# yurimjeon1892/EFGH

Hardware: AMD Instinct MI355X
Metric: frame-pairs/sec EFGHNet fwd+bwd (384x1280 RGB + 64x2048 range), whole job (higher is better)
Workload: dtype f32; 1 GPU; BASELINE.json configs[2]: EFGHNet fwd+bwd with efghloss + gradient all-reduce + fused Adam, synthetic 384x1280 RGB + 131072-point sweep, batch=8 per GPU, random-init weights; global_batch=8, points=131072, parallelism=dp1

## Files before the change

### efgh_amd/_C.py

```python
import ctypes
import os

_HERE = os.path.dirname(os.path.abspath(__file__))
SO_PATH = os.environ.get('EFGH_LIB') or os.path.join(_HERE, 'lib', 'libefgh_hip.so')
_lib = None
ABI_VERSION = 4

c_void_p, c_int, c_int32, c_int64, c_float = (ctypes.c_void_p, ctypes.c_int, ctypes.c_int32,
                                              ctypes.c_int64, ctypes.c_float)


class EfghError(RuntimeError):
    pass


class GemmDesc(ctypes.Structure):
    _fields_ = [
        ('A', c_void_p), ('lda', c_int64), ('C', c_int32), ('T', c_int32), ('mode', c_int32),
        ('B', c_int32), ('Hin', c_int32), ('Win', c_int32), ('Hv', c_int32), ('Wv', c_int32),
        ('sh', c_int32), ('sw', c_int32),
        ('dh', ctypes.c_int8 * 16), ('dw', ctypes.c_int8 * 16),
        ('Ho', c_int32), ('Wo', c_int32), ('osh', c_int32), ('osw', c_int32), ('oh0', c_int32),
        ('ow0', c_int32),
        ('table', c_void_p), ('W', c_void_p), ('N', c_int32), ('M', c_int64), ('M_dev', c_void_p),
        ('bias', c_void_p), ('scale', c_void_p), ('shift', c_void_p),
        ('residual', c_void_p), ('ldr', c_int64),
        ('act', c_int32), ('slope', c_float), ('out', c_void_p), ('ldo', c_int64),
        ('stats', c_void_p),
        ('nbatch', c_int32), ('batch_stride_a', c_int64), ('batch_stride_w', c_int64), ('batch_stride_out', c_int64),
        ('batch_stride_table', c_int32), ('table_alias_mask', c_int32),
        ('stats_mode', c_int32), ('bn_raw', c_void_p), ('bn_ldraw', c_int64), ('bn_y', c_void_p), ('bn_ldy', c_int64),
        ('bn_pscale', c_void_p), ('bn_pshift', c_void_p), ('bn_mean', c_void_p), ('bn_invstd', c_void_p),
        ('bn_act', c_int32), ('bn_slope', c_float),
    ]


class WgradOutDesc(ctypes.Structure):
    _fields_ = [('W', c_void_p), ('N', c_int32), ('T', c_int32), ('C', c_int32), ('Cp', c_int32),
                ('sn', c_int64), ('sc', c_int64), ('st', c_int64), ('taps', c_int32 * 16), ('accumulate', c_int32)]


GUARD_MAX_SEGMENTS = 8
GUARD_RUN = 4096


class GuardState(ctypes.Structure):
    _fields_ = [('sumsq', ctypes.c_double * GUARD_MAX_SEGMENTS), ('sumsq_total', ctypes.c_double), ('norm', ctypes.c_double),
                ('nonfinite', c_int64 * GUARD_MAX_SEGMENTS), ('nonfinite_total', c_int64),
                ('applied', c_int64), ('skipped', c_int64),
                ('coef', c_float), ('scale', c_float), ('bc1', c_float), ('bc2_sqrt', c_float),
                ('skip', c_int32), ('nseg', c_int32)]


class TxnState(ctypes.Structure):
    _fields_ = [('forward_nonfinite', c_int64), ('rolled_back', c_int64), ('vetoed_total', c_int64),
                ('first_bad', c_int32), ('vetoed', c_int32)]


WROTE_OUT = 1


def check_wrote(rc):
    if rc == WROTE_OUT:
        return True
    check(rc)
    return False


def lib():
    global _lib
    if _lib is None:
        if not os.path.exists(SO_PATH):
            raise EfghError(f'{SO_PATH} is missing: run `python -c "import __graft_entry__ as g; '
                            f'g.build()"` (hipcc, gfx950). There is no CPU fallback.')
        import torch
        _lib = ctypes.CDLL(SO_PATH)
        _lib.efgh_last_error.restype = ctypes.c_char_p
        _lib.efgh_version.restype = c_int
        if _lib.efgh_version() != ABI_VERSION:
            got, _lib = _lib.efgh_version(), None
            raise EfghError(f'{SO_PATH} has ABI version {got}, this package binds version {ABI_VERSION} of include/efgh_hip.h: '
                            f'rebuild it (`python -m efgh_amd.build`)')
        _lib.efgh_wino2d_tiles.restype = c_int64
        _lib.efgh_segment_workspace.restype = c_int64
        _lib.efgh_gather_wgrad_workspace.restype = c_int64
        _lib.efgh_plane_wgrad_workspace.restype = c_int64
        _lib.efgh_wino_wgrad_workspace.restype = c_int64
        _lib.efgh_sc_wgrad_workspace.restype = c_int64
        _lib.efgh_c4n4_wgrad_workspace.restype = c_int64
        _lib.efgh_c4_wgrad_workspace.restype = c_int64
        _lib.efgh_thin_wgrad_workspace.restype = c_int64
        _lib.efgh_lattice_hash_capacity.restype = c_int64
        _lib.efgh_lattice_hash_capacity.argtypes = [c_int32]
        _lib.efgh_lattice_workspace_bytes.restype = c_int64
        _lib.efgh_lattice_workspace_bytes.argtypes = [c_int32, c_int32, c_int32]
        _lib.efgh_lattice_part_max_entries.argtypes = [c_int32]
        _lib.efgh_lattice_part_buckets.argtypes = [c_int32]
        _lib.efgh_lattice_part_list_len.restype = c_int64
        _lib.efgh_lattice_part_list_len.argtypes = [c_int32, c_int32]
        _lib.efgh_lattice_part_zeroed_bytes.restype = c_int64
        _lib.efgh_lattice_part_zeroed_bytes.argtypes = [c_int32]
        _lib.efgh_lattice_part_workspace_bytes.restype = c_int64
        _lib.efgh_lattice_part_workspace_bytes.argtypes = [c_int32, c_int32, c_int32, c_int32, c_int32]
        _lib.efgh_lattice_neighbors_r_workspace.restype = c_int64
        _lib.efgh_lattice_neighbors_r_workspace.argtypes = [c_int32, c_int32]
        _lib.efgh_lattice_index_bytes.restype = c_int64
        _lib.efgh_lattice_index_bytes.argtypes = [c_int32, c_int32]
        _lib.efgh_offsets_invert_workspace.restype = c_int64
        _lib.efgh_offsets_invert_workspace.argtypes = [c_int32, c_int32]
        _lib.efgh_slice_bwd_workspace.restype = c_int64
        _lib.efgh_slice_bwd_workspace.argtypes = [c_int32]
        _lib.efgh_grad_guard_workspace.restype = c_int64
        _lib.efgh_grad_guard_workspace.argtypes = [c_int64]
        _lib.efgh_grad_guard_measure.argtypes = [c_void_p, c_int64, ctypes.POINTER(c_int64), c_int32, ctypes.c_double, c_float,
                                                 c_int32, c_float, c_float, c_int32, c_void_p, c_void_p, c_int32, c_void_p]
        _lib.efgh_adam_step_guarded.argtypes = [c_void_p, c_void_p, c_void_p, c_void_p, c_int64, c_float, c_float, c_float,
                                                c_float, c_float, c_void_p, c_void_p]
        _lib.efgh_grad_drain.argtypes = [c_void_p, c_void_p, c_int64, c_int32, c_void_p]
        _lib.efgh_gimg_valid_count.argtypes = [c_void_p, c_void_p, c_int32, c_int64, c_void_p, c_void_p]
        _lib.efgh_txn_snapshot.argtypes = [c_void_p, c_void_p, c_int64, c_void_p, c_void_p, c_int64, c_void_p, c_void_p]
        _lib.efgh_txn_probe.argtypes = [c_void_p, c_void_p, c_int64, c_void_p, c_int32, c_void_p, c_int32, c_int64, c_void_p,
                                        c_void_p]
        _lib.efgh_txn_resolve.argtypes = [c_void_p, c_void_p, c_int64, c_void_p, c_void_p, c_int64, c_void_p, c_void_p, c_float,
                                          c_float, c_void_p]
    return _lib


def check(rc):
    if rc != 0:
        raise EfghError(f'libefgh_hip: rc={rc}: {lib().efgh_last_error().decode()}')


def ptr(t):
    return c_void_p(0 if t is None else t.data_ptr())


_raw_stream = None


def stream_ptr():
    global _raw_stream
    import torch
    if _raw_stream is None:
        get, dev = getattr(torch._C, '_cuda_getCurrentRawStream', None), getattr(torch._C, '_cuda_getDevice', None)
        if get is not None and dev is not None:
            _raw_stream = lambda: get(dev())
        else:
            _raw_stream = lambda: torch.cuda.current_stream().cuda_stream
    return c_void_p(_raw_stream())


def require_cuda(*tensors):
    for t in tensors:
        if t is not None and not t.is_cuda:
            raise EfghError('efgh_amd runs on the GPU through libefgh_hip.so only (got a CPU tensor); '
                            'there is no CPU fallback')


def require_f32(*tensors):
    import torch
    for t in tensors:
        if t is not None and t.dtype != torch.float32:
            raise EfghError('efgh_amd expects float32 tensors, got %s (cast with .float() as iterater.py:29-32 does)' % t.dtype)
```

### efgh_amd/csrc/wgrad.hip

```cpp
#include "common.h"

namespace {

typedef float f32x16 __attribute__((ext_vector_type(16)));
constexpr int TK = 128, TM = 32, LD = 128;

struct WArgs {
    const float *A; int64_t lda;
    int C, T, K;
    unsigned magicC;
    int Hin, Win, Hv, Wv, sh, sw;
    unsigned long long dhpack, dwpack;
    int Ho, Wo, osh, osw, oh0, ow0;
    const int *table;
    const float *G; int64_t ldg;
    int N;
    int tld;
    long long M; int mchunk;
    float *dW;
    long long zstride;
    unsigned kt, nt;
    long long bsA, bsG, bsD;
};

// ... 64 lines not shown
    }
    float4 rg[NGQ], ra[4];
    auto load_step = [&](long long ms) {
        if (TN != 128) {
#pragma unroll
            for (int q = 0; q < NGQ; ++q) {
                long long m = ms + gr0 + GRS * q;
                float4 g = make_float4(0.f, 0.f, 0.f, 0.f);
                if (m < mend && nin) g = *reinterpret_cast<const float4 *>(MODE == 1 ? git[q].g : p.G + m * p.ldg + n0 + gc4);
                rg[q] = g;
                if (MODE == 1) advance(git[q], n0 + gc4);
            }
        }
#pragma unroll
        for (int q = 0; q < 4; ++q) {
            long long m = ms + r0 + 8 * q;
            float4 g = make_float4(0.f, 0.f, 0.f, 0.f), a = g;
            if (m < mend) {
                if (MODE == 1) {
                    if (TN == 128 && nin) g = *reinterpret_cast<const float4 *>(rit[q].g);
                    if (kin && rit[q].rowok && (unsigned)(rit[q].j * p.sw + dw) < (unsigned)p.Win)
                        a = *reinterpret_cast<const float4 *>(rit[q].a);
                } else {
                    long long arow = -1;
                    if (MODE == 0) arow = m;
                    else if (kin) arow = p.table[m * (MODE == 4 ? p.tld : 16) + t];
                    if (TN == 128 && nin) g = *reinterpret_cast<const float4 *>(p.G + m * p.ldg + n0 + c4);
                    if (kin && arow >= 0) a = *reinterpret_cast<const float4 *>(p.A + arow * p.lda + c);
                }
            }
            if (TN == 128) rg[q] = g;
            ra[q] = a;
            if (MODE == 1) advance(rit[q], n0 + c4);
        }
    };

    f32x16 acc[2][TJ];
#pragma unroll
    for (int i = 0; i < 2; ++i)
#pragma unroll
        for (int j = 0; j < TJ; ++j)
#pragma unroll
            for (int r = 0; r < 16; ++r) acc[i][j][r] = 0.f;

    load_step(mbeg);
    for (long long ms = mbeg; ms < mend; ms += TM) {
#pragma unroll
        for (int q = 0; q < 4; ++q)
            *reinterpret_cast<float4 *>(&As[(r0 + 8 * q) * LD + c4]) = ra[q];
#pragma unroll
        for (int q = 0; q < NGQ; ++q)
            *reinterpret_cast<float4 *>(&Gs[(gr0 + GRS * q) * TN + gc4]) = rg[q];
        __syncthreads();
        if (ms + TM < mend) load_step(ms + TM);
#pragma unroll
        for (int mm = 0; mm < TM / 2; ++mm) {
            float g[2], a[TJ];
#pragma unroll
            for (int i = 0; i < 2; ++i) g[i] = Gs[(mm * 2 + lh) * TN + (wn * 2 + i) * 32 + l31];
#pragma unroll
            for (int j = 0; j < TJ; ++j) a[j] = As[(mm * 2 + lh) * LD + (wk * TJ + j) * 32 + l31];
#pragma unroll
            for (int i = 0; i < 2; ++i)
#pragma unroll
                for (int j = 0; j < TJ; ++j)
                    acc[i][j] = __builtin_amdgcn_mfma_f32_32x32x2f32(g[i], a[j], acc[i][j], 0, 0, 0);
        }
        __syncthreads();
    }
#pragma unroll
    for (int i = 0; i < 2; ++i)
#pragma unroll
        for (int j = 0; j < TJ; ++j) {
            const int k = k0 + (wk * TJ + j) * 32 + l31;
            if (k >= p.K) continue;
#pragma unroll
            for (int r = 0; r < 16; ++r) {
                const int n = n0 + (wn * 2 + i) * 32 + (r & 3) + 8 * (r >> 2) + 4 * lh;
                if (n < p.N) p.dW[(long long)n * p.K + k] = acc[i][j][r];
            }
        }
}

typedef efgh_wgrad_out_desc FoldUnpackArgs;

template <bool UNPACK>
__global__ void __launch_bounds__(256) k_fold_splits(const float4 *part, int zs, long long total4, float4 *dst, const FoldUnpackArgs u) {
    __shared__ float4 red[256];
    const int e = threadIdx.x & 15, zl = threadIdx.x >> 4;
    const long long i = (long long)blockIdx.x * 16 + e;
    float4 a = make_float4(0.f, 0.f, 0.f, 0.f), b = a;
    if (i < total4) {
        int z = zl;
        for (; z + 16 < zs; z += 32) {
            const float4 u = part[(long long)z * total4 + i], v = part[(long long)(z + 16) * total4 + i];
            a.x += u.x; a.y += u.y; a.z += u.z; a.w += u.w;
            b.x += v.x; b.y += v.y; b.z += v.z; b.w += v.w;
        }
        if (z < zs) { const float4 u = part[(long long)z * total4 + i]; a.x += u.x; a.y += u.y; a.z += u.z; a.w += u.w; }
        a.x += b.x; a.y += b.y; a.z += b.z; a.w += b.w;
    }
    red[threadIdx.x] = a;
    __syncthreads();
    for (int h = 8; h; h >>= 1) {
        if (zl < h) {
            const float4 o = red[threadIdx.x + h * 16];
            float4 m = red[threadIdx.x];
            m.x += o.x; m.y += o.y; m.z += o.z; m.w += o.w;
            red[threadIdx.x] = m;
        }
        __syncthreads();
    }
    if (zl == 0 && i < total4) {
        if (!UNPACK) { dst[i] = red[e]; return; }
        const float4 v4 = red[e];
        const float v[4] = {v4.x, v4.y, v4.z, v4.w};
        const long long idx = 4 * i;
        const int c0 = (int)(idx % u.Cp); const long long r = idx / u.Cp;
        const int t = (int)(r % u.T), n = (int)(r / u.T);
        if (n >= u.N) return;
        int ti = 0;
#pragma unroll
        for (int q = 0; q < 16; ++q) if (q == t) ti = u.taps[q];
#pragma unroll
        for (int q = 0; q < 4; ++q) {
            if (c0 + q >= u.C) continue;
            float *d = &u.W[n * u.sn + (c0 + q) * u.sc + ti * u.st];
            *d = u.accumulate ? *d + v[q] : v[q];
        }
    }
}

__global__ void k_unpack_weight(const float *__restrict__ Wp, float *__restrict__ W, int N, int T, int C,
                                int Cp, long long sn, long long sc, long long st, const int4 taps0,
                                const int4 taps1, const int4 taps2, const int4 taps3, int accumulate) {
    const int tp[16] = {taps0.x, taps0.y, taps0.z, taps0.w, taps1.x, taps1.y, taps1.z, taps1.w,
                        taps2.x, taps2.y, taps2.z, taps2.w, taps3.x, taps3.y, taps3.z, taps3.w};
    long long total = (long long)N * T * C;
    for (long long i = (long long)blockIdx.x * blockDim.x + threadIdx.x; i < total;
         i += (long long)gridDim.x * blockDim.x) {
        int c = (int)(i % C); long long r = i / C;
        int t = (int)(r % T); int n = (int)(r / T);
        int ti = 0;
#pragma unroll
        for (int q = 0; q < 16; ++q) if (q == t) ti = tp[q];
        float v = Wp[((long long)n * T + t) * Cp + c];
        float *dst = &W[n * sn + c * sc + ti * st];
        *dst = accumulate ? *dst + v : v;
    }
}

__global__ void __launch_bounds__(256)
k_table_scatter_add(const float *__restrict__ src, const int *__restrict__ table, long long M, int T, int C,
                    float *__restrict__ dst) {
    const int c4n = C >> 2;
    long long total = M * T * c4n;
    for (long long i = (long long)blockIdx.x * 256 + threadIdx.x; i < total; i += (long long)gridDim.x * 256) {
        int cq = (int)(i % c4n); long long r = i / c4n;
        int t = (int)(r % T); long long m = r / T;
        int row = table[m * 16 + t];
        if (row < 0) continue;
        float4 v = *reinterpret_cast<const float4 *>(src + (m * T + t) * C + cq * 4);
        float *d = dst + (long long)row * C + cq * 4;
        atomicAdd(d + 0, v.x); atomicAdd(d + 1, v.y); atomicAdd(d + 2, v.z); atomicAdd(d + 3, v.w);
    }
}

}

bool efgh_launch_fold_splits(const float *part, int zs, long long total, float *dst, hipStream_t st, const efgh_wgrad_out_desc *out) {
    const long long total4 = total / 4;
    const unsigned grid = (unsigned)((total4 + 15) / 16);
    if (out && out->W && out->T >= 1 && out->T <= 16 && out->Cp >= out->C && out->Cp % 4 == 0) {
        const long long row = (long long)out->T * out->Cp;
        if (total % row == 0 && total / row >= out->N && total / row < out->N + 4) {
            k_fold_splits<true><<<grid, 256, 0, st>>>((const float4 *)part, zs, total4, (float4 *)dst, *out);
            return true;
        }
    }
    FoldUnpackArgs none = {};
    k_fold_splits<false><<<grid, 256, 0, st>>>((const float4 *)part, zs, total4, (float4 *)dst, none);
    return false;
}

static int gather_wgrad_impl(const efgh_gemm_desc *d, const float *G, int64_t ldg, float *dWp, float *workspace, int nbatch,
                             int64_t bsG, int64_t bsD, const efgh_wgrad_out_desc *out, void *stream_, int tld = 0);


static long long wgrad_chunks(const efgh_gemm_desc *d, int nbatch, long long *chunk_out) {
    const int K = d->T * d->C;
    const int TN = d->N <= 64 ? 64 : 128;
    const long long kt = (K + TK - 1) / TK, nt = (d->N + TN - 1) / TN;
    static const int occ128[3] = {efgh_wg_per_cu((const void *)k_gather_wgrad<0, 128>, 256, 0), efgh_wg_per_cu((const void *)k_gather_wgrad<1, 128>, 256, 0),
                                  efgh_wg_per_cu((const void *)k_gather_wgrad<2, 128>, 256, 0)};
    static const int occ64[3] = {efgh_wg_per_cu((const void *)k_gather_wgrad<0, 64>, 256, 0), efgh_wg_per_cu((const void *)k_gather_wgrad<1, 64>, 256, 0),
                                 efgh_wg_per_cu((const void *)k_gather_wgrad<2, 64>, 256, 0)};
    const int mode = d->mode >= 0 && d->mode <= 2 ? d->mode : 0;
    return efgh_round_chunks(d->M, kt * nt * nbatch, TN == 128 ? occ128[mode] : occ64[mode], TM, 256, (double)nbatch * d->N * K, chunk_out);
}

extern "C" int64_t efgh_gather_wgrad_workspace(const efgh_gemm_desc *d) {
    if (!d || d->C <= 0 || d->T < 1 || d->N < 1 || d->M < 1) return 0;
    const int nbatch = d->nbatch > 1 ? d->nbatch : 1;
    const long long zs = wgrad_chunks(d, nbatch, nullptr);
    return zs > 1 ? zs * nbatch * (int64_t)d->N * d->T * d->C : 0;
}

extern "C" int efgh_gather_wgrad(const efgh_gemm_desc *d, const float *G, int64_t ldg, float *dWp, float *workspace,
                                 const efgh_wgrad_out_desc *out, void *stream_) {
    return gather_wgrad_impl(d, G, ldg, dWp, workspace, 1, 0, 0, out, stream_);
}

extern "C" int efgh_gather_wgrad_batched(const efgh_gemm_desc *d, const float *G, int64_t ldg, int64_t batch_stride_g,
                                         float *dWp, int64_t batch_stride_dw, float *workspace, void *stream_) {
    EFGH_CHECK_ARG(d && d->mode == 0 && d->nbatch >= 1 && d->nbatch <= 65535);
    EFGH_CHECK_ARG(d->batch_stride_a % 4 == 0 && batch_stride_g % 4 == 0 && batch_stride_dw == (int64_t)d->N * d->C);
    return gather_wgrad_impl(d, G, ldg, dWp, workspace, d->nbatch, batch_stride_g, batch_stride_dw, nullptr, stream_);
}

static int gather_wgrad_impl(const efgh_gemm_desc *d, const float *G, int64_t ldg, float *dWp, float *workspace, int nbatch,
                             int64_t bsG, int64_t bsD, const efgh_wgrad_out_desc *out, void *stream_, int tld) {
    hipStream_t st = (hipStream_t)stream_;
    EFGH_CHECK_ARG(d && d->A && G && dWp);
    EFGH_CHECK_ARG(d->C > 0 && d->C % 4 == 0 && d->T >= 1 && (d->T <= 16 || tld > 0) && d->N >= 1 && d->M >= 1);
    EFGH_CHECK_ARG(tld == 0 || (d->mode == 2 && d->table != nullptr && tld >= d->T && nbatch == 1 && !out));
    EFGH_CHECK_ARG(d->lda % 4 == 0 && ldg % 4 == 0 && d->N % 4 == 0);
    EFGH_CHECK_ARG((((uintptr_t)d->A) & 15) == 0 && (((uintptr_t)G) & 15) == 0 && (((uintptr_t)dWp) & 15) == 0);
    EFGH_CHECK_ARG((int64_t)d->T * d->C < 65536 && d->mode >= 0 && d->mode <= 2);
    WArgs a;
    a.A = d->A; a.lda = d->lda; a.C = d->C; a.T = d->T; a.K = d->T * d->C;
    a.magicC = (unsigned)((0x100000000ULL + d->C - 1) / d->C);
    a.Hin = d->Hin; a.Win = d->Win; a.Hv = d->Hv; a.Wv = d->Wv; a.sh = d->sh; a.sw = d->sw;
    a.dhpack = 0; a.dwpack = 0;
    for (int t = 0; t < 16; ++t) {
        int dh = t < d->T ? d->dh[t] : 0, dw = t < d->T ? d->dw[t] : 0;
        a.dhpack |= (unsigned long long)((dh + 8) & 15) << (4 * t);
        a.dwpack |= (unsigned long long)((dw + 8) & 15) << (4 * t);
    }
    a.Ho = d->Ho; a.Wo = d->Wo; a.osh = d->osh; a.osw = d->osw; a.oh0 = d->oh0; a.ow0 = d->ow0;
    a.table = d->table; a.G = G; a.ldg = ldg; a.N = d->N; a.M = d->M;
    a.bsA = nbatch > 1 ? d->batch_stride_a : 0; a.bsG = bsG; a.bsD = bsD; a.tld = tld;
    if (d->mode == 1) EFGH_CHECK_ARG(d->M == (int64_t)d->B * d->Hv * d->Wv && d->osh >= 1 && d->osw >= 1);
    if (d->mode == 2) EFGH_CHECK_ARG(d->table != nullptr);
    const int TN = a.N <= 64 ? 64 : 128;
    const int kt = (a.K + TK - 1) / TK, nt = (a.N + TN - 1) / TN;
    long long chunk = 0;
    const long long zs = wgrad_chunks(d, nbatch, &chunk);
    a.mchunk = (int)chunk;
    EFGH_CHECK_ARG(zs * kt * nt < 0x7fffffffLL);
    a.kt = (unsigned)kt; a.nt = (unsigned)nt;
    const long long plane = (long long)nbatch * a.N * a.K;
    EFGH_CHECK_ARG(zs == 1 || (workspace && (((uintptr_t)workspace) & 15) == 0));
    a.dW = zs > 1 ? workspace : dWp;
    a.zstride = zs > 1 ? plane : 0;
    const dim3 grid((unsigned)(zs * kt * nt), (unsigned)nbatch);
    if (tld > 0) {
        if (TN == 128) k_gather_wgrad<4, 128><<<grid, 256, 0, st>>>(a);
        else k_gather_wgrad<4, 64><<<grid, 256, 0, st>>>(a);
    } else if (TN == 128) {
        if (d->mode == 0) k_gather_wgrad<0, 128><<<grid, 256, 0, st>>>(a);
        else if (d->mode == 1) k_gather_wgrad<1, 128><<<grid, 256, 0, st>>>(a);
        else k_gather_wgrad<2, 128><<<grid, 256, 0, st>>>(a);
    } else {
        if (d->mode == 0) k_gather_wgrad<0, 64><<<grid, 256, 0, st>>>(a);
        else if (d->mode == 1) k_gather_wgrad<1, 64><<<grid, 256, 0, st>>>(a);
        else k_gather_wgrad<2, 64><<<grid, 256, 0, st>>>(a);
    }
    bool wrote = false;
    if (zs > 1) wrote = efgh_launch_fold_splits(workspace, (int)zs, plane, dWp, st, nbatch == 1 ? out : nullptr);
    EFGH_CHECK_LAUNCH();
    return wrote ? EFGH_WROTE_OUT : EFGH_OK;
}

extern "C" int efgh_blur_r_wgrad(const efgh_gemm_desc *d, int32_t ld, const float *G, int64_t ldg, float *dWp, float *workspace,
                                 void *stream_) {
    EFGH_CHECK_ARG(ld > 0);
    const int rc = gather_wgrad_impl(d, G, ldg, dWp, workspace, 1, 0, 0, nullptr, stream_, ld);
    return rc == EFGH_WROTE_OUT ? EFGH_OK : rc;
}

extern "C" int efgh_unpack_weight(const float *Wp, float *W, int32_t N, int32_t T, int32_t C, int32_t Cp,
                                  int64_t sn, int64_t sc, int64_t stt, const int32_t *tapidx, int32_t accumulate,
                                  void *stream_) {
    EFGH_CHECK_ARG(Wp && W && N > 0 && T > 0 && T <= 16 && C > 0 && Cp >= C);
    int tp[16];
    for (int t = 0; t < 16; ++t) tp[t] = (tapidx && t < T) ? tapidx[t] : (t < T ? t : 0);
    long long total = (long long)N * T * C;
    int grid = (int)((total + 255) / 256);
    if (grid > 8192) grid = 8192;
    k_unpack_weight<<<grid, 256, 0, (hipStream_t)stream_>>>(Wp, W, N, T, C, Cp, sn, sc, stt,
                                                           make_int4(tp[0], tp[1], tp[2], tp[3]),
                                                           make_int4(tp[4], tp[5], tp[6], tp[7]),
                                                           make_int4(tp[8], tp[9], tp[10], tp[11]),
                                                           make_int4(tp[12], tp[13], tp[14], tp[15]), accumulate);
    EFGH_CHECK_LAUNCH();
    return EFGH_OK;
}

extern "C" int efgh_table_scatter_add(const float *src, const int32_t *table, int64_t M, int32_t T, int32_t C,
                                      float *dst, void *stream_) {
    EFGH_CHECK_ARG(src && table && dst && M > 0 && T > 0 && T <= 16 && C % 4 == 0);
    long long total = M * T * (C / 4);
    long long g = (total + 255) / 256;
    k_table_scatter_add<<<(int)(g > 16384 ? 16384 : g), 256, 0, (hipStream_t)stream_>>>(src, table, M, T, C, dst);
    EFGH_CHECK_LAUNCH();
    return EFGH_OK;
}

extern "C" int efgh_debug_occupancy(char *out, int32_t cap) {
    EFGH_CHECK_ARG(out && cap > 64);
    snprintf(out, cap, "k_gather_wgrad<0,128> %d  <1,128> %d  <2,128> %d  <0,64> %d  <1,64> %d  <2,64> %d workgroups per CU",
             efgh_wg_per_cu((const void *)k_gather_wgrad<0, 128>, 256, 0), efgh_wg_per_cu((const void *)k_gather_wgrad<1, 128>, 256, 0),
             efgh_wg_per_cu((const void *)k_gather_wgrad<2, 128>, 256, 0), efgh_wg_per_cu((const void *)k_gather_wgrad<0, 64>, 256, 0),
             efgh_wg_per_cu((const void *)k_gather_wgrad<1, 64>, 256, 0), efgh_wg_per_cu((const void *)k_gather_wgrad<2, 64>, 256, 0));
    return EFGH_OK;
}
```

### efgh_amd/ops.py

```python
import ctypes
import os as _os
import threading
import weakref

import torch

from . import _C
from ._C import c_float, c_int32, c_int64, ptr

ACT_NONE, ACT_RELU, ACT_LEAKY = 0, 1, 2


def _L():
    return _C.lib()


def _st():
    return _C.stream_ptr()


def ceil4(n):
    return (n + 3) // 4 * 4


# ... 542 lines not shown
    def regroup():
        return Wp.view(N, S, Ts * C).permute(1, 0, 2).contiguous()
    Wg = _cached(Wp, ('ksplit', S), _ver(Wp), regroup)
    part = _scratch(S * M * N, dev)
    gather_gemm(A, lda, C, Ts, Wg, N, M, part, N, mode=2, table=table, a_off=a_off, batch=(S, 0, N * Ts * C, M * N, Ts),
                flops=flops if flops is not None else 2.0 * M * N * 15 * C, alias_mask=alias_mask)
    b = None
    if bias is not None:
        b = bias if bias.numel() == N else None
        assert b is not None
    _C.check(_L().efgh_fold_planes(ptr(part), c_int32(S), c_int64(M), c_int32(N), ptr(b), c_int32(act), c_float(slope),
                                   _C.c_void_p(out.data_ptr() + 4 * out_off), c_int64(ldo), _st()))


def gather_gemm(A, lda, C, T, Wp, N, M, out, ldo, mode=0, geom=None, table=None, bias=None, scale=None,
                shift=None, residual=None, ldr=0, act=ACT_NONE, slope=0.0, stats=None, a_off=0, out_off=0,
                res_off=0, M_dev=None, flops=None, batch=None, alias_mask=False, bn_bwd=None, pool=False, lazy=None, pre_v=None):
    key = (mode, C, N, T, geom, M, stats is not None, M_dev is not None, batch is not None, pool,
           scale is None and shift is None and residual is None and (bias is None or bias.numel() == N))
    route = gemm_route(*key)
    if (lazy is not None or pre_v is not None) and not (route == 'wino2d' and min(C, N) >= 64):
        raise _C.EfghError('gather_gemm(lazy= / pre_v=) on a launch the 2-D Winograd path does not serve (ask lazy_capable() first)')
    if route == 'blur_r':
        if (geom is not None or batch is not None or M_dev is not None or scale is not None or shift is not None or residual is not None
                or stats is not None or alias_mask or pool or bn_bwd is not None):
            raise _C.EfghError('gather_gemm(mode=MODE_BLUR_R) takes a plain blur launch: bias and activation only')
        blur_r_gemm(A, lda, C, T, Wp, N, M, out, ldo, table, bias=bias, act=act, slope=slope, a_off=a_off, out_off=out_off, flops=flops)
        return None
    if route == 'ksplit':
        return _blur_gemm_ksplit(A, lda, C, Wp, N, M, out, ldo, table, bias, act, slope, a_off, out_off, flops, alias_mask)
    d = _desc(A, lda, C, T, mode, N, M, geom, table, a_off, Wp, out, ldo, out_off, bias, scale, shift, residual, ldr, res_off, act, slope,
              stats, M_dev, batch)
    d.table_alias_mask = 1 if (alias_mask and mode == 2) else 0
    if route == 'sc' and not _sc_aligned(d, lda, ldo, residual, ldr, stats):
        route = gemm_route(*key, aligned=False)
    if pool and route not in ('c4', 'wino2d', 'wino_hpool'):
        raise _C.EfghError('gather_gemm(pool=True) on a launch no pooling epilogue serves (ask pool_fusable() first)')
    ev = _prof_start(PROFILE)
    bn_stats = None
    if route == 'thin':
        if TRACE_THIN is not None:
            TRACE_THIN.append(int(_L().efgh_thin_supported(ctypes.byref(d))))
        _C.check(_L().efgh_thin_gemm(ctypes.byref(d), _st()))
    elif route == 'c4':
        assert lda % 4 == 0
        _C.check((_L().efgh_c4_conv3x3_pooled if pool else _L().efgh_c4_conv3x3)(ctypes.byref(d), _st()))
    elif route == 'sc':
        _C.check(_L().efgh_sc_conv3x3(ctypes.byref(d), _st()))
    elif route == 'wino2d':
        if (bn_bwd is not None and stats is None and BN_BWD_FUSED_2D and out_off == 0 and not pool and bn_bwd.fits(M, N)
                and bn_bwd.y is None and bn_bwd.raw.stride(-2) % 4 == 0):
            rows = _L().efgh_wino2d_stats_rows(c_int32(geom[0]), c_int32(geom[1]), c_int32(geom[2]), c_int32(N))
            bn_stats = _bn_bwd_sums(d, bn_bwd, rows, N, out.device)
        _wino2d_forward(d, A, a_off, lda, C, N, geom, Wp, pool=pool, lazy=lazy, pre_v=pre_v)
    elif route == 'wino_hpool':
        _C.check(_L().efgh_wino_conv3x3_hpool(ctypes.byref(d), ptr(wino_weight(Wp, N, C)), _st()))
    elif route == 'wino':
        if bn_bwd is not None and stats is None and BN_BWD_FUSED and out_off == 0 and bn_bwd.fits(M, N):
            rows = _L().efgh_wino_grid_m(c_int32(geom[0]), c_int32(geom[1]), c_int32(geom[2]))
            bn_stats = _bn_bwd_sums(d, bn_bwd, rows, N, out.device)
        _C.check(_L().efgh_wino_conv3x3(ctypes.byref(d), ptr(wino_weight(Wp, N, C)), _st()))
    else:
        _C.check(_L().efgh_gather_gemm(ctypes.byref(d), _st()))
    if ev is not None:
        _prof_end(ev, route, (mode, M, N, T, C), float(flops) if flops is not None else 2.0 * M * N * T * C, PROFILE, PROFILE_WINO,
                  batched=batch is not None)
    return bn_stats


def _bn_bwd_sums(d, src, rows, N, device):
    part = torch.empty((rows, 2, N), dtype=torch.float32, device=device)
    d.stats, d.stats_mode = part.data_ptr(), 1
    d.bn_raw, d.bn_ldraw = src.raw.data_ptr(), src.raw.stride(-2)
    if src.y is not None:
        d.bn_y, d.bn_ldy = src.y.data_ptr(), src.y.stride(-2)
    else:
        d.bn_pscale, d.bn_pshift = src.psc.data_ptr(), src.psh.data_ptr()
    d.bn_mean, d.bn_invstd = src.mean.data_ptr(), src.invstd.data_ptr()
    d.bn_act, d.bn_slope = src.act, src.slope
    return part


GEMM_DMA = True


def apply_switches():
    _L().efgh_gather_gemm_set_dma(c_int32(1 if GEMM_DMA else 0))


PLANE_DMA = True
PLANE_DMA_NBUF = 0
PROFILE_WINO2D = None
PROFILE_WINO2D_GEMM = None
PLANES_SPLIT = None
PLANE_SPLIT_HITS = [0, 0]


def planes_split_active():
    if PLANES_SPLIT is not None:
        return bool(PLANES_SPLIT)
    return torch.backends.cuda.matmul.fp32_precision == 'tf32'


def _planes_split_now():
    m = TLS.planes_split
    return planes_split_active() if m is None else m


def _batched_plain_gemm(A3, W3, out3, rows, C, N):
    g = _desc(A3, 36 * C, C, 1, 0, N, rows, Wp=W3, out=out3, ldo=36 * N, batch=(36, C, N * C, N))
    ev = _prof_start(PROFILE_WINO2D_GEMM)
    if PLANE_DMA and _L().efgh_plane_gemm_supported(ctypes.byref(g)):
        if _planes_split_now():
            PLANE_SPLIT_HITS[0] += 1
            _C.check(_L().efgh_plane_gemm_x6(ctypes.byref(g), c_int32(PLANE_DMA_NBUF), _st()))
        else:
            _C.check(_L().efgh_plane_gemm(ctypes.byref(g), c_int32(PLANE_DMA_NBUF), _st()))
    else:
        _C.check(_L().efgh_gather_gemm(ctypes.byref(g), _st()))
    _prof_end(ev, 'planes', (0, rows, N, 36, C), 2.0 * 36 * rows * C * N, PROFILE_WINO2D_GEMM)


W2V_CACHE = {}
W2V_KEEP = True


def w2v_clear():
    me = threading.get_ident()
    with _LOCK:
        for k in [k for k, v in W2V_CACHE.items() if v[2] == me]:
            del W2V_CACHE[k]


POOL_FUSED = True
POOL_HALF = True


def pool_fusable(mode, C, N, geom, residual=None, stats=None):
    if not (POOL_FUSED and residual is None and stats is None and geom is not None and geom[1] >= 2 and geom[2] >= 2):
        return False
    route = gemm_route(mode, C, N, len(geom[7]), geom, geom[0] * geom[3] * geom[4], pool='h')
    if route == 'c4':
        return geom[5] == 1 and geom[6] == 1
    if route == 'wino2d':
        return True
    return 'h' if (route == 'wino_hpool' and POOL_HALF) else False


class LazyAct:
    __slots__ = ('scale', 'shift', 'act', 'slope')

    def __init__(self, scale, shift, act, slope):
        self.scale, self.shift, self.act, self.slope = scale, shift, act, slope


LAZY_ACT = True
W2_BWD_FUSED = True
W2_BWD_FUSED_POOL = True
LAZY_HITS = [0, 0]


def lazy_capable(mode, C, N, geom):
    return geom is not None and min(C, N) >= 64 and gemm_route(mode, C, N, len(geom[7]), geom, 0) == 'wino2d'


def wino2d_input(A, a_off, lda, C, B, H, W, V, lazy=None):
    if lazy is None:
        _C.check(_L().efgh_wino2d_input(_C.c_void_p(A.data_ptr() + 4 * a_off), c_int64(lda), c_int32(C), c_int32(B), c_int32(H),
                                        c_int32(W), ptr(V), _st()))
    else:
# ... 891 lines not shown
```

### include/efgh_hip.h

```cpp
#ifndef EFGH_HIP_H
#define EFGH_HIP_H
#include <stdint.h>

#ifdef __cplusplus
extern "C" {
#endif

#define EFGH_OK 0
#define EFGH_E_INVALID (-1)
#define EFGH_E_LAUNCH (-2)
#define EFGH_WROTE_OUT 1

const char *efgh_last_error(void);

#define EFGH_ABI_VERSION 4
int efgh_version(void);

#define EFGH_LATTICE_INFO_H 0
#define EFGH_LATTICE_INFO_ERR 1
#define EFGH_LATTICE_INFO_ALIAS 2
#define EFGH_LATTICE_INFO_CURSOR 3
#define EFGH_LATTICE_INFO_SEG 4
#define EFGH_LATTICE_MAX_SAMPLES 1024

// ... 241 lines not shown
                             void *stream);
int efgh_softmax2_bwd(const float *y, const float *dy, int32_t B, int64_t HW, float *dx, int64_t ld, void *stream);
int efgh_heads_bwd(const float *y, const float *dmask, const float *ddepth, int32_t B, int64_t HW, float *dx, void *stream);
int efgh_corr1d_bwd(const float *rp, const float *cam, const float *cam_mm, const float *dlogit, int32_t B,
                    int32_t h, int32_t wc, int32_t wp, float *dcam_n, float *drp, void *stream);
int efgh_corr_unpad(const float *drp, int32_t B, int32_t h, int32_t w, int32_t C, int32_t off, float *dx,
                    void *stream);

int efgh_adam_step(float *w, const float *g, float *m, float *v, int64_t n, float lr, float beta1,
                   float beta2, float eps, float weight_decay, int32_t step, float grad_scale, void *stream);

#define EFGH_GUARD_MAX_SEGMENTS 8
#define EFGH_GUARD_RUN 4096
typedef struct efgh_guard_state {
    double sumsq[EFGH_GUARD_MAX_SEGMENTS];
    double sumsq_total;
    double norm;
    int64_t nonfinite[EFGH_GUARD_MAX_SEGMENTS];
    int64_t nonfinite_total;
    int64_t applied;
    int64_t skipped;
    float coef;
    float scale;
    float bc1;
    float bc2_sqrt;
    int32_t skip;
    int32_t nseg;
} efgh_guard_state;
int64_t efgh_grad_guard_workspace(int64_t n);
int efgh_grad_guard_measure(const float *g, int64_t n, const int64_t *bounds, int32_t nseg, double max_norm, float grad_scale,
                            int32_t skip_nonfinite, float beta1, float beta2, int32_t step, void *workspace,
                            efgh_guard_state *state, int32_t grid, void *stream);
int efgh_adam_step_guarded(float *w, const float *g, float *m, float *v, int64_t n, float lr, float beta1, float beta2,
                           float eps, float weight_decay, const efgh_guard_state *state, void *stream);

int efgh_grad_drain(float *acc, float *g, int64_t n, int32_t first, void *stream);
int efgh_gimg_valid_count(const float *gdep4, const uint8_t *img_mask, int32_t B, int64_t HW, int64_t *count, void *stream);

typedef struct efgh_txn_state {
    int64_t forward_nonfinite;
    int64_t rolled_back;
    int64_t vetoed_total;
    int32_t first_bad;
    int32_t vetoed;
} efgh_txn_state;
int efgh_txn_snapshot(const float *live_f, float *shadow_f, int64_t nf, const int64_t *live_c, int64_t *shadow_c, int64_t nc,
                      efgh_txn_state *txn, void *stream);
int efgh_txn_probe(const float *live_f, const float *shadow_f, int64_t nf, const int64_t *starts, int32_t nseg, const float *losses,
                   int32_t k, int64_t loss_stride, efgh_txn_state *txn, void *stream);
int efgh_txn_resolve(float *live_f, const float *shadow_f, int64_t nf, int64_t *live_c, const int64_t *shadow_c, int64_t nc,
                     efgh_guard_state *guard, efgh_txn_state *txn, float beta1, float beta2, void *stream);

int efgh_thin_supported(const efgh_gemm_desc *d);
int efgh_thin_gemm(const efgh_gemm_desc *d, void *stream);
int64_t efgh_thin_wgrad_workspace(const efgh_gemm_desc *d);
int efgh_thin_wgrad(const efgh_gemm_desc *d, const float *G, int64_t ldg, float *dWp, float *workspace,
                    const efgh_wgrad_out_desc *out, void *stream);
int efgh_c4n4_supported(const efgh_gemm_desc *d);
int64_t efgh_c4n4_wgrad_workspace(const efgh_gemm_desc *d);
int efgh_c4n4_wgrad(const efgh_gemm_desc *d, const float *G, int64_t ldg, float *dWp, float *workspace,
                    const efgh_wgrad_out_desc *out, void *stream);

int efgh_sc_supported(const efgh_gemm_desc *d);
int32_t efgh_sc_stats_rows(int32_t B, int32_t H, int32_t W);
int efgh_sc_conv3x3(const efgh_gemm_desc *d, void *stream);
int efgh_sc_wgrad_supported(const efgh_gemm_desc *d);
int64_t efgh_sc_wgrad_workspace(const efgh_gemm_desc *d);
int efgh_sc_wgrad(const efgh_gemm_desc *d, const float *G, int64_t ldg, float *dWp, float *workspace,
                  const efgh_wgrad_out_desc *out, void *stream);
int efgh_c4_supported(const efgh_gemm_desc *d);
int32_t efgh_c4_stats_rows(int32_t B, int32_t Ho, int32_t Wo);
int efgh_c4_conv3x3(const efgh_gemm_desc *d, void *stream);
int efgh_c4_pooled_supported(const efgh_gemm_desc *d);
int efgh_c4_conv3x3_pooled(const efgh_gemm_desc *d, void *stream);
int efgh_c4_wgrad_supported(const efgh_gemm_desc *d);
int64_t efgh_c4_wgrad_workspace(const efgh_gemm_desc *d);
int efgh_c4_wgrad(const efgh_gemm_desc *d, const float *G, int64_t ldg, float *dWp, float *workspace,
                  const efgh_wgrad_out_desc *out, void *stream);

int efgh_debug_occupancy(char *out, int32_t cap);

int efgh_gather_gemm_set_dma(int32_t on);

int efgh_plane_gemm_supported(const efgh_gemm_desc *d);
int efgh_plane_gemm(const efgh_gemm_desc *d, int32_t nbuf, void *stream);
int efgh_plane_wgrad_supported(const efgh_gemm_desc *d, int64_t ldg);
int64_t efgh_plane_wgrad_workspace(const efgh_gemm_desc *d);
int efgh_plane_wgrad_batched(const efgh_gemm_desc *d, const float *G, int64_t ldg, int64_t batch_stride_g, float *dWp,
                             int64_t batch_stride_dw, float *workspace, int32_t nbuf, void *stream);

int efgh_plane_gemm_x6(const efgh_gemm_desc *d, int32_t nbuf, void *stream);
int efgh_plane_wgrad_x6_batched(const efgh_gemm_desc *d, const float *G, int64_t ldg, int64_t batch_stride_g, float *dWp,
                                int64_t batch_stride_dw, float *workspace, int32_t nbuf, void *stream);

int efgh_convt_col2im(const float *Y, int64_t ldy, int32_t B, int32_t Hin, int32_t Win, int32_t Ho, int32_t Wo,
                      int32_t O, int32_t pad, const float *scale, const float *shift, int32_t act, float slope,
                      float *out, int64_t ldo, void *stream);
int efgh_convt_im2col(const float *G, int64_t ldg, int32_t B, int32_t Hin, int32_t Win, int32_t Ho, int32_t Wo,
                      int32_t O, int32_t pad, float *Ycol, int64_t ldy, void *stream);

int efgh_corr_pack_cam(const float *cam, const float *cam_mm, int32_t B, int32_t h, int32_t wc, int32_t segw,
                       int32_t nseg, int32_t nsplit, float *Wc, void *stream);
int efgh_corr_fold(const float *P, int32_t B, int32_t nsplit, int64_t Mv, int32_t ldp, int32_t nseg, int32_t segw,
                   int32_t nj, float *logit, float *score, void *stream);
int efgh_norm_bwd(const float *x, const float *dxn, const float *mm, int32_t B, int64_t n, float *part, float *dx, void *stream);
int efgh_corr_planes(const float *x, const float *mm, int32_t B, int32_t h, int32_t w, int32_t w_in_pitch, int32_t wP,
                     float *out, void *stream);
int efgh_corr_unplanes(const float *in, int32_t B, int32_t h, int32_t w, int32_t wP, float *out, void *stream);
int efgh_corr_toeplitz(const float *dl, int32_t B, int32_t nj, int32_t rows, int32_t cols, int32_t colsP, int32_t transpose,
                       float *T, void *stream);

int efgh_wino_supported(const efgh_gemm_desc *d);
int32_t efgh_wino_grid_m(int32_t B, int32_t H, int32_t W);
int efgh_wino_pack(const float *Wp, float *U, int32_t N, int32_t C, void *stream);
int efgh_wino_conv3x3_hpool(const efgh_gemm_desc *d, const float *U, void *stream);
int efgh_wino_conv3x3(const efgh_gemm_desc *d, const float *U, void *stream);
int efgh_wino_wgrad_supported(const efgh_gemm_desc *d);
int64_t efgh_wino_wgrad_workspace(const efgh_gemm_desc *d);
int efgh_wino_wgrad(const efgh_gemm_desc *d, const float *G, int64_t ldg, float *S, float *dWp, const efgh_wgrad_out_desc *out,
                    void *stream);

int efgh_prep_affine_nearest_u8(const uint8_t *in, int32_t h, int32_t w, const int64_t *coef6_host, uint8_t *out,
                                int32_t nh, int32_t nw, void *stream);
int efgh_prep_crop_pad_u8(const uint8_t *in, int32_t h, int32_t w, int32_t oy, int32_t ox, uint8_t *out, int32_t th,
                          int32_t tw, void *stream);
int efgh_prep_resample_u8(const uint8_t *in, int32_t h, int32_t w, int32_t axis, int32_t out_size, const int32_t *bounds,
                          const int32_t *coeffs, int32_t ksize, uint8_t *out, void *stream);
int efgh_prep_hwc_to_chw_u8(const uint8_t *in, int32_t h, int32_t w, uint8_t *chw, uint8_t *mask, void *stream);
int efgh_prep_u8_to_f32_chw_pad(const uint8_t *in, int32_t h, int32_t w, int32_t oy, int32_t ox, float *out, int32_t th,
                                int32_t tw, void *stream);
int32_t efgh_prep_filter_blocks(int32_t n);
int efgh_prep_radius_filter(const float *pcd, const int32_t *pre_idx, int32_t n, int32_t flip_xy, float radius,
                            int32_t *block_scratch, int32_t *keep_idx, int32_t *count, void *stream);
int efgh_prep_gather_transform(const float *pcd, const int32_t *keep_idx, const int32_t *sel, int32_t n_sel,
                               int32_t flip_xy, const double *T34, int32_t num_points, float *out32, double *out64,
                               void *stream);

int efgh_pose_errors(const float *gt, const float *pred, int32_t B, int32_t mode, float *rot_err, float *trs_err,
                     void *stream);

int32_t efgh_gimg_loss_groups(int64_t n);
int efgh_gimg_loss_fwd(const float *pred_depth, const float *pred_mask, int64_t mask_bstride, const float *gdep4,
                       const uint8_t *img_mask, int32_t B, int64_t HW, float *gt_depth, float *gt_mask, double *part,
                       float *out3, void *stream);
int efgh_gimg_loss_bwd(const float *pred_depth, const float *pred_mask, int64_t mask_bstride, const float *gt_depth,
                       const uint8_t *img_mask, int32_t B, int64_t HW, const float *sums3, const float *g_depth,
                       const float *g_mask, float *d_pred_depth, float *d_pred_mask, int64_t dmask_bstride, void *stream);

int efgh_sum_depth_last(const float *pc, int64_t pc_cstride, int32_t N, const double *T34, int32_t H, int32_t W, int32_t *idx_ws,
                        uint8_t *out, void *stream);
int efgh_sum_range_last(const float *pc, int64_t pc_cstride, int32_t N, const double *T34, int32_t H, int32_t W, double fov_up,
                        double fov_down, int32_t *idx_ws, double *out, void *stream);
int efgh_sum_paint(const void *jobs_dev, int32_t njobs, void *stream);
int efgh_sum_colorize(const double *minmax, int64_t n, const uint8_t *lut, uint8_t *rgb, uint8_t *mask, void *stream);

int efgh_pose_head_normal(const float *abs_logits, int64_t lda, const float *sgn_logits, int64_t lds, int32_t B, int32_t nd,
                          float dx, float dy, float dz, float *abs_out, float *normal, float *R44, void *stream);
int efgh_pose_head_yaw(const float *score, int64_t lds, int32_t B, int32_t n, float *R44, void *stream);
int efgh_pose_cam_T_velo(const float *c_T, int64_t ldc, const float *l_T, const float *calib, const float *A, int32_t B,
                         float *out34, void *stream);

int efgh_pose_head_normal_bwd(const float *abs_logits, int64_t lda, const float *sgn_logits, int64_t lds, int32_t B, int32_t nd,
                              float dx, float dy, float dz, const float *g_abs, const float *g_normal, const float *g_R44,
                              float *g_abs_logits, void *stream);
int efgh_pose_mat44_mul(const float *a, const float *b, int32_t B, int32_t transpose_a, int32_t transpose_b, float *out, void *stream);
int efgh_pose_rotation_between(const float *src3, int32_t B, float dx, float dy, float dz, float *R44, void *stream);
// ... 23 lines not shown
```

Before: 31.07 frame-pairs/s.

## Add DMA-ring pipelined gather weight-gradient kernel with multi-buffered LDS staging

Adds a new weight-gradient GEMM kernel that stages the gathered activation and output-gradient tiles into a two- or three-slot LDS ring through direct global-to-LDS loads, then runs MFMA over the staged tile while later stages are still loading. It is enabled by default for strided-gather mode 1 with specific tap counts, and occupancy-based chunking now accounts for the ring's LDS footprint. The aim is to hide global-load latency in the wgrad reductions. In exchange it uses more LDS per workgroup, which can lower occupancy, and it adds zero-source padding and more index bookkeeping.

Measured after the change: 31.12 frame-pairs/s, median of 3. Within noise of the previous version (+0.1%).

```diff
diff --git a/efgh_amd/_C.py b/efgh_amd/_C.py
--- a/efgh_amd/_C.py
+++ b/efgh_amd/_C.py
@@ -85,6 +85,8 @@
         _lib.efgh_segment_workspace.restype = c_int64
         _lib.efgh_gather_wgrad_workspace.restype = c_int64
         _lib.efgh_plane_wgrad_workspace.restype = c_int64
+        _lib.efgh_gather_wgrad_set_dma.restype = c_int
+        _lib.efgh_gather_wgrad_set_dma.argtypes = [c_int32]
         _lib.efgh_wino_wgrad_workspace.restype = c_int64
         _lib.efgh_sc_wgrad_workspace.restype = c_int64
         _lib.efgh_c4n4_wgrad_workspace.restype = c_int64
diff --git a/efgh_amd/csrc/wgrad.hip b/efgh_amd/csrc/wgrad.hip
--- a/efgh_amd/csrc/wgrad.hip
+++ b/efgh_amd/csrc/wgrad.hip
@@ -170,6 +170,158 @@
         }
 }
 
+__device__ __attribute__((aligned(512))) float g_wgrad_zero[128];
+
+constexpr int TMS = 16;
+
+template <int MODE, int TN, int NBUF>
+__global__ void __launch_bounds__(256)
+k_gather_wgrad_dma(const WArgs p0) {
+    constexpr int TJ = TN == 128 ? 2 : 1;
+    constexpr int NPA = TMS / 8;
+    constexpr int NPG = TMS * TN / 1024;
+    constexpr int NPER = NPA + NPG;
+    constexpr int STAGE = TMS * (TN + LD);
+    extern __shared__ __attribute__((aligned(1024))) float wring[];
+    WArgs p = p0;
+    p.A += (long long)blockIdx.y * p0.bsA; p.G += (long long)blockIdx.y * p0.bsG; p.dW += (long long)blockIdx.y * p0.bsD;
+    const int tid = threadIdx.x, lane = tid & 63, wave = __builtin_amdgcn_readfirstlane(tid >> 6);
+    const int wn = TN == 128 ? (wave >> 1) : 0, wk = TN == 128 ? (wave & 1) : wave;
+    const int l31 = lane & 31, lh = lane >> 5;
+    const unsigned ring_lds = lds_addr(wring);
+    const unsigned nblk = gridDim.x, q8 = nblk >> 3, r8 = nblk & 7, xcd = blockIdx.x & 7, within = blockIdx.x >> 3;
+    const unsigned lin = (xcd < r8 ? xcd * (q8 + 1) : r8 * (q8 + 1) + (xcd - r8) * q8) + within;
+    const unsigned per_z = p.kt * p.nt, bz = lin / per_z, rem = lin - bz * per_z;
+    const unsigned by = rem / p.kt, bx = rem - by * p.kt;
+    const int k0 = bx * TK, n0 = by * TN;
+    const long long mbeg = (long long)bz * p.mchunk;
+    long long mend = mbeg + p.mchunk;
+    if (mend > p.M) mend = p.M;
+    if (mbeg >= mend) return;
+    p.dW += (long long)bz * p.zstride;
+
+    const int c4 = l31 * 4, kk = k0 + c4;
+    const bool kin = kk < p.K;
+    const int t = (int)(((unsigned long long)kk * p.magicC) >> 32);
+    const int c = kk - t * p.C;
+    const int dh = (int)((p.dhpack >> (4 * (t & 15))) & 15) - 8, dw = (int)((p.dwpack >> (4 * (t & 15))) & 15) - 8;
+    const int gc4 = TN == 128 ? c4 : (lane & 15) * 4;
+    const bool nin = (n0 + gc4) < p.N;
+    const float *zsrc = g_wgrad_zero + c4;
+
+    struct RowIt { int j, i; long long b; const float *g, *a; bool rowok; };
+    auto point = [&](RowIt &it, int gcol) {
+        const long long orow = (it.b * p.Ho + (it.i * p.osh + p.oh0)) * p.Wo + (it.j * p.osw + p.ow0);
+        it.g = p.G + orow * p.ldg + gcol;
+        const int ih = it.i * p.sh + dh;
+        it.rowok = (unsigned)ih < (unsigned)p.Hin;
+        it.a = p.A + ((it.b * p.Hin + ih) * p.Win + (it.j * p.sw + dw)) * p.lda + c;
+    };
+    auto place = [&](RowIt &it, long long m, int gcol) {
+        if (MODE == 0) { it.g = p.G + m * p.ldg + gcol; it.a = p.A + m * p.lda + c; return; }
+        it.j = (int)(m % p.Wv); const long long r = m / p.Wv;
+        it.i = (int)(r % p.Hv); it.b = r / p.Hv;
+        point(it, gcol);
+    };
+    const long long gstep = (long long)TMS * (MODE == 1 ? p.osw : 1) * p.ldg, astep = (long long)TMS * (MODE == 1 ? p.sw : 1) * p.lda;
+    const bool narrow = p.Wv < 4 * TMS;
+    auto advance = [&](RowIt &it, int gcol) {
+        it.g += gstep; it.a += astep;
+        if (MODE == 0) return;
+        it.j += TMS;
+        if (narrow || it.j >= p.Wv) {
+            while (it.j >= p.Wv) { it.j -= p.Wv; ++it.i; }
+            while (it.i >= p.Hv) { it.i -= p.Hv; ++it.b; }
+            point(it, gcol);
+        }
+    };
+    RowIt rit[NPA], git[NPG];
+#pragma unroll
+    for (int q = 0; q < NPA; ++q) place(rit[q], mbeg + (wave * NPA + q) * 2 + lh, n0 + c4);
+    if (TN != 128) {
+#pragma unroll
+        for (int q = 0; q < NPG; ++q) place(git[q], mbeg + (wave * NPG + q) * 4 + (lane >> 4), n0 + gc4);
+    }
+    auto issue = [&](long long ms, int buf) {
+        const unsigned base = ring_lds + (unsigned)(buf * STAGE) * 4u;
+        if (TN != 128) {
+#pragma unroll
+            for (int q = 0; q < NPG; ++q) {
+                const long long m = ms + (wave * NPG + q) * 4 + (lane >> 4);
+                dma16(m < mend && nin ? git[q].g : zsrc, base + (unsigned)(wave * NPG + q) * 1024u);
+                advance(git[q], n0 + gc4);
+            }
+        }
+#pragma unroll
+        for (int q = 0; q < NPA; ++q) {
+            const long long m = ms + (wave * NPA + q) * 2 + lh;
+            const bool in = m < mend;
+            if (TN == 128) dma16(in && nin ? rit[q].g : zsrc, base + (unsigned)(wave * NPA + q) * 1024u);
+            bool aok = in && kin;
+            if (MODE == 1) aok = aok && rit[q].rowok && (unsigned)(rit[q].j * p.sw + dw) < (unsigned)p.Win;
+            dma16(aok ? rit[q].a : zsrc, base + (unsigned)(TMS * TN) * 4u + (unsigned)(wave * NPA + q) * 1024u);
+            advance(rit[q], n0 + c4);
+        }
+    };
+
+    f32x16 acc[2][TJ];
+#pragma unroll
+    for (int i = 0; i < 2; ++i)
+#pragma unroll
+        for (int j = 0; j < TJ; ++j)
+#pragma unroll
+            for (int r = 0; r < 16; ++r) acc[i][j][r] = 0.f;
+
+    const int nst = (int)((mend - mbeg + TMS - 1) / TMS);
+#pragma unroll
+    for (int s = 0; s < NBUF - 1; ++s)
+        if (s < nst) issue(mbeg + (long long)s * TMS, s);
+    const int gx = lh * TN + wn * 64 + 2 * l31;
+    const int ax = TMS * TN + lh * LD + (TN == 128 ? wk * 64 + 2 * l31 : wk * 32 + l31);
+    int slot = 0, fill = NBUF - 1;
+    for (int s = 0; s < nst; ++s) {
+        if (NBUF == 2 || s + 1 >= nst) wait_vm<0>();
+        else wait_vm<NPER>();
+        __builtin_amdgcn_s_barrier();
+        asm volatile("" ::: "memory");
+        if (s + NBUF - 1 < nst) issue(mbeg + (long long)(s + NBUF - 1) * TMS, fill);
+        const float *S = wring + slot * STAGE;
+        slot = slot + 1 == NBUF ? 0 : slot + 1;
+        fill = fill + 1 == NBUF ? 0 : fill + 1;
+        float2 g[2], a[2];
+        auto frag = [&](int mm, float2 &fg, float2 &fa) {
+            fg = *reinterpret_cast<const float2 *>(S + mm * 2 * TN + gx);
+            if (TN == 128) fa = *reinterpret_cast<const float2 *>(S + mm * 2 * LD + ax);
+            else fa.x = S[mm * 2 * LD + ax];
+        };
+        frag(0, g[0], a[0]);
+#pragma unroll
+        for (int mm = 0; mm < TMS / 2; ++mm) {
+            if (mm + 1 < TMS / 2) frag(mm + 1, g[(mm + 1) & 1], a[(mm + 1) & 1]);
+            __builtin_amdgcn_sched_barrier(0);
+            const float2 cg = g[mm & 1], ca = a[mm & 1];
+            acc[0][0] = __builtin_amdgcn_mfma_f32_32x32x2f32(cg.x, ca.x, acc[0][0], 0, 0, 0);
+            if (TN == 128) acc[0][TJ - 1] = __builtin_amdgcn_mfma_f32_32x32x2f32(cg.x, ca.y, acc[0][TJ - 1], 0, 0, 0);
+            acc[1][0] = __builtin_amdgcn_mfma_f32_32x32x2f32(cg.y, ca.x, acc[1][0], 0, 0, 0);
+            if (TN == 128) acc[1][TJ - 1] = __builtin_amdgcn_mfma_f32_32x32x2f32(cg.y, ca.y, acc[1][TJ - 1], 0, 0, 0);
+            __builtin_amdgcn_sched_barrier(0);
+        }
+    }
+#pragma unroll
+    for (int q = 0; q < 2; ++q) {
+        const int k = k0 + (TN == 128 ? wk * 64 + 2 * l31 : wk * 32 + l31);
+        if (k >= p.K) continue;
+#pragma unroll
+        for (int r = 0; r < 16; ++r) {
+            const int n = n0 + wn * 64 + 2 * ((r & 3) + 8 * (r >> 2) + 4 * lh) + q;
+            if (n >= p.N) continue;
+            float *dp = p.dW + (long long)n * p.K + k;
+            if (TN == 128) *reinterpret_cast<float2 *>(dp) = make_float2(acc[q][0][r], acc[q][TJ - 1][r]);
+            else *dp = acc[q][0][r];
+        }
+    }
+}
+
 typedef efgh_wgrad_out_desc FoldUnpackArgs;
 
 template <bool UNPACK>
@@ -275,7 +427,23 @@
                              int64_t bsG, int64_t bsD, const efgh_wgrad_out_desc *out, void *stream_, int tld = 0);
 
 
-static long long wgrad_chunks(const efgh_gemm_desc *d, int nbatch, long long *chunk_out) {
+static int g_wgrad_dma = 1;
+
+static inline size_t wgrad_dma_lds(int TN, int nbuf) { return (size_t)nbuf * TMS * (TN + LD) * sizeof(float); }
+
+static bool wgrad_dma_class_ok(int mode, int TN, int T) {
+    if (mode != 1) return false;
+    return TN == 128 ? (T == 2 || T == 4 || T == 9) : T == 1;
+}
+
+static bool wgrad_dma_ok(const efgh_gemm_desc *d, int tld) {
+    if (!g_wgrad_dma || tld > 0 || (d->mode != 0 && d->mode != 1)) return false;
+    if (d->lda % 4 || d->C % 4 || (((uintptr_t)d->A) & 15)) return false;
+    if (g_wgrad_dma >= 2) return true;
+    return wgrad_dma_class_ok(d->mode, d->N <= 64 ? 64 : 128, d->T);
+}
+
+static long long wgrad_chunks(const efgh_gemm_desc *d, int nbatch, long long *chunk_out, int tld = 0) {
     const int K = d->T * d->C;
     const int TN = d->N <= 64 ? 64 : 128;
     const long long kt = (K + TK - 1) / TK, nt = (d->N + TN - 1) / TN;
@@ -283,8 +451,15 @@
                                   efgh_wg_per_cu((const void *)k_gather_wgrad<2, 128>, 256, 0)};
     static const int occ64[3] = {efgh_wg_per_cu((const void *)k_gather_wgrad<0, 64>, 256, 0), efgh_wg_per_cu((const void *)k_gather_wgrad<1, 64>, 256, 0),
                                  efgh_wg_per_cu((const void *)k_gather_wgrad<2, 64>, 256, 0)};
+    static const int occ_dma[2][2][2] = {
+        {{efgh_wg_per_cu((const void *)k_gather_wgrad_dma<0, 64, 3>, 256, wgrad_dma_lds(64, 3)), efgh_wg_per_cu((const void *)k_gather_wgrad_dma<0, 128, 3>, 256, wgrad_dma_lds(128, 3))},
+         {efgh_wg_per_cu((const void *)k_gather_wgrad_dma<1, 64, 3>, 256, wgrad_dma_lds(64, 3)), efgh_wg_per_cu((const void *)k_gather_wgrad_dma<1, 128, 3>, 256, wgrad_dma_lds(128, 3))}},
+        {{efgh_wg_per_cu((const void *)k_gather_wgrad_dma<0, 64, 2>, 256, wgrad_dma_lds(64, 2)), efgh_wg_per_cu((const void *)k_gather_wgrad_dma<0, 128, 2>, 256, wgrad_dma_lds(128, 2))},
+         {efgh_wg_per_cu((const void *)k_gather_wgrad_dma<1, 64, 2>, 256, wgrad_dma_lds(64, 2)), efgh_wg_per_cu((const void *)k_gather_wgrad_dma<1, 128, 2>, 256, wgrad_dma_lds(128, 2))}}};
     const int mode = d->mode >= 0 && d->mode <= 2 ? d->mode : 0;
-    return efgh_round_chunks(d->M, kt * nt * nbatch, TN == 128 ? occ128[mode] : occ64[mode], TM, 256, (double)nbatch * d->N * K, chunk_out);
+    int occ = TN == 128 ? occ128[mode] : occ64[mode];
+    if (wgrad_dma_ok(d, tld)) occ = occ_dma[g_wgrad_dma == 2][mode][TN == 128];
+    return efgh_round_chunks(d->M, kt * nt * nbatch, occ, TM, 256, (double)nbatch * d->N * K, chunk_out);
 }
 
 extern "C" int64_t efgh_gather_wgrad_workspace(const efgh_gemm_desc *d) {
@@ -333,7 +508,7 @@
     const int TN = a.N <= 64 ? 64 : 128;
     const int kt = (a.K + TK - 1) / TK, nt = (a.N + TN - 1) / TN;
     long long chunk = 0;
-    const long long zs = wgrad_chunks(d, nbatch, &chunk);
+    const long long zs = wgrad_chunks(d, nbatch, &chunk, tld);
     a.mchunk = (int)chunk;
     EFGH_CHECK_ARG(zs * kt * nt < 0x7fffffffLL);
     a.kt = (unsigned)kt; a.nt = (unsigned)nt;
@@ -342,7 +517,27 @@
     a.dW = zs > 1 ? workspace : dWp;
     a.zstride = zs > 1 ? plane : 0;
     const dim3 grid((unsigned)(zs * kt * nt), (unsigned)nbatch);
-    if (tld > 0) {
+    if (wgrad_dma_ok(d, tld)) {
+        const int nbuf = g_wgrad_dma == 2 ? 2 : 3;
+        const size_t lds = wgrad_dma_lds(TN, nbuf);
+        if (nbuf == 3) {
+            if (TN == 128) {
+                if (d->mode == 0) k_gather_wgrad_dma<0, 128, 3><<<grid, 256, lds, st>>>(a);
+                else k_gather_wgrad_dma<1, 128, 3><<<grid, 256, lds, st>>>(a);
+            } else {
+                if (d->mode == 0) k_gather_wgrad_dma<0, 64, 3><<<grid, 256, lds, st>>>(a);
+                else k_gather_wgrad_dma<1, 64, 3><<<grid, 256, lds, st>>>(a);
+            }
+        } else {
+            if (TN == 128) {
+                if (d->mode == 0) k_gather_wgrad_dma<0, 128, 2><<<grid, 256, lds, st>>>(a);
+                else k_gather_wgrad_dma<1, 128, 2><<<grid, 256, lds, st>>>(a);
+            } else {
+                if (d->mode == 0) k_gather_wgrad_dma<0, 64, 2><<<grid, 256, lds, st>>>(a);
+                else k_gather_wgrad_dma<1, 64, 2><<<grid, 256, lds, st>>>(a);
+            }
+        }
+    } else if (tld > 0) {
         if (TN == 128) k_gather_wgrad<4, 128><<<grid, 256, 0, st>>>(a);
         else k_gather_wgrad<4, 64><<<grid, 256, 0, st>>>(a);
     } else if (TN == 128) {
@@ -395,11 +590,23 @@
     return EFGH_OK;
 }
 
+extern "C" int efgh_gather_wgrad_set_dma(int32_t on) {
+    const int old = g_wgrad_dma;
+    g_wgrad_dma = on == 2 || on == 3 ? on : (on != 0 ? 1 : 0);
+    return old;
+}
+
 extern "C" int efgh_debug_occupancy(char *out, int32_t cap) {
     EFGH_CHECK_ARG(out && cap > 64);
-    snprintf(out, cap, "k_gather_wgrad<0,128> %d  <1,128> %d  <2,128> %d  <0,64> %d  <1,64> %d  <2,64> %d workgroups per CU",
+    int n = snprintf(out, cap, "k_gather_wgrad<0,128> %d  <1,128> %d  <2,128> %d  <0,64> %d  <1,64> %d  <2,64> %d workgroups per CU",
              efgh_wg_per_cu((const void *)k_gather_wgrad<0, 128>, 256, 0), efgh_wg_per_cu((const void *)k_gather_wgrad<1, 128>, 256, 0),
              efgh_wg_per_cu((const void *)k_gather_wgrad<2, 128>, 256, 0), efgh_wg_per_cu((const void *)k_gather_wgrad<0, 64>, 256, 0),
              efgh_wg_per_cu((const void *)k_gather_wgrad<1, 64>, 256, 0), efgh_wg_per_cu((const void *)k_gather_wgrad<2, 64>, 256, 0));
+    if (n > 0 && n < cap)
+        snprintf(out + n, cap - n, "\nk_gather_wgrad_dma (three-slot ring) <0,128> %d  <1,128> %d  <0,64> %d  <1,64> %d | (two-slot ring) <0,128> %d  <1,128> %d  <0,64> %d  <1,64> %d",
+                 efgh_wg_per_cu((const void *)k_gather_wgrad_dma<0, 128, 3>, 256, wgrad_dma_lds(128, 3)), efgh_wg_per_cu((const void *)k_gather_wgrad_dma<1, 128, 3>, 256, wgrad_dma_lds(128, 3)),
+                 efgh_wg_per_cu((const void *)k_gather_wgrad_dma<0, 64, 3>, 256, wgrad_dma_lds(64, 3)), efgh_wg_per_cu((const void *)k_gather_wgrad_dma<1, 64, 3>, 256, wgrad_dma_lds(64, 3)),
+                 efgh_wg_per_cu((const void *)k_gather_wgrad_dma<0, 128, 2>, 256, wgrad_dma_lds(128, 2)), efgh_wg_per_cu((const void *)k_gather_wgrad_dma<1, 128, 2>, 256, wgrad_dma_lds(128, 2)),
+                 efgh_wg_per_cu((const void *)k_gather_wgrad_dma<0, 64, 2>, 256, wgrad_dma_lds(64, 2)), efgh_wg_per_cu((const void *)k_gather_wgrad_dma<1, 64, 2>, 256, wgrad_dma_lds(64, 2)));
     return EFGH_OK;
 }
diff --git a/efgh_amd/ops.py b/efgh_amd/ops.py
--- a/efgh_amd/ops.py
+++ b/efgh_amd/ops.py
@@ -648,10 +648,12 @@
 
 
 GEMM_DMA = True
+WGRAD_DMA = True
 
 
 def apply_switches():
     _L().efgh_gather_gemm_set_dma(c_int32(1 if GEMM_DMA else 0))
+    _L().efgh_gather_wgrad_set_dma(c_int32(int(WGRAD_DMA)))
 
 
 PLANE_DMA = True
diff --git a/include/efgh_hip.h b/include/efgh_hip.h
--- a/include/efgh_hip.h
+++ b/include/efgh_hip.h
@@ -347,6 +347,8 @@
 
 int efgh_gather_gemm_set_dma(int32_t on);
 
+int efgh_gather_wgrad_set_dma(int32_t on);
+
 int efgh_plane_gemm_supported(const efgh_gemm_desc *d);
 int efgh_plane_gemm(const efgh_gemm_desc *d, int32_t nbuf, void *stream);
 int efgh_plane_wgrad_supported(const efgh_gemm_desc *d, int64_t ldg);
```
